# PereUbu7/Variational-Self-Organizing-Maps

Measured on AMD Instinct MI355X. Metric: training samples/sec per epoch (BMU+update), 128x128 map, 784-dim, higher is better.
Workload: dtype f32

## Files before the change

### include/vsom_hip.h

```cpp
#ifndef VSOM_HIP_H
#define VSOM_HIP_H

#include <stddef.h>
#include <stdint.h>

#ifdef __cplusplus
extern "C" {
#endif

typedef struct vsom_ctx vsom_ctx;

typedef enum vsom_status {
    VSOM_OK = 0,
    VSOM_ERR_INVALID = -1,
    VSOM_ERR_HIP = -2,
    VSOM_ERR_NOMEM = -3,
    VSOM_ERR_UNSUPPORTED = -4
} vsom_status;

typedef enum vsom_transform {
    VSOM_STANDARD = 0,
    VSOM_MEDIAN = 1,
    VSOM_CLR = 2
} vsom_transform;
// ... 52 lines not shown
                uint32_t in_len, int transform);
void vsom_destroy(vsom_ctx *ctx);

#define VSOM_CUSTOM_MAX_DEPTH 5120
int vsom_create_custom(vsom_ctx **out, int device, uint32_t width, uint32_t height, uint32_t in_len,
                       uint32_t depth, uint32_t residual_len, const char *hook_source);
int vsom_custom_compile_check(const char *hook_source, uint32_t depth, uint32_t residual_len);
int vsom_set_column_weights(vsom_ctx *ctx, const float *weights_host );
int vsom_set_chunk_validity(vsom_ctx *ctx, const uint8_t *valid_host, int one_mask);
int vsom_find_bmu_valid(vsom_ctx *ctx, const float *v_host, const uint8_t *valid_host , uint64_t *bmu_out,
                        float *dist_out);
int vsom_find_local_bmu_valid(vsom_ctx *ctx, const float *v_host, const uint8_t *valid_host, uint64_t last_bmu,
                              uint64_t *bmu_out, float *dist_out);
int vsom_dist_single_valid(vsom_ctx *ctx, const float *v_host, const uint8_t *valid_host, uint64_t node, float *dist_out);
int vsom_train_single_valid(vsom_ctx *ctx, const float *v_host, const uint8_t *valid_host, double eta, double sigma,
                            uint64_t *last_bmu, int decay_fn, float *residual_out, float *dist_out, uint64_t *bmu_out);
int vsom_set_stream(vsom_ctx *ctx, void *hip_stream);
int vsom_synchronize(vsom_ctx *ctx);
int vsom_set_bmu_mode(vsom_ctx *ctx, int mode);
int vsom_set_update_mode(vsom_ctx *ctx, int mode);
int vsom_set_sigma_mode(vsom_ctx *ctx, int mode);
int vsom_sigma_flush(vsom_ctx *ctx);
int vsom_sigma_stats(vsom_ctx *ctx, uint64_t *out );
int vsom_set_column_compaction(vsom_ctx *ctx, long min_rows);
int vsom_set_row_dedupe(vsom_ctx *ctx, double min_work);
int vsom_get_shortlist_stats(vsom_ctx *ctx, uint32_t *out );
uint32_t vsom_depth(const vsom_ctx *ctx);
uint32_t vsom_nodes(const vsom_ctx *ctx);

int vsom_set_state(vsom_ctx *ctx, const float *map, const float *sigma, const float *S,
                   const float *weight, const uint64_t *bmu_hits);
int vsom_get_state(vsom_ctx *ctx, float *map, float *sigma, float *S, float *weight,
                   uint64_t *bmu_hits);

int vsom_upload_chunk(vsom_ctx *ctx, const float *x_host, size_t B);
int vsom_upload_chunk_async(vsom_ctx *ctx, const float *x_host, size_t B);
int vsom_set_chunk_device(vsom_ctx *ctx, const float *x_dev, size_t B);
int vsom_host_alloc(void **out, size_t bytes);
int vsom_host_free(void *p);
int vsom_prefetch_chunk(vsom_ctx *ctx, const float *x_host, size_t B);
int vsom_prefetch_wait(vsom_ctx *ctx);
int vsom_commit_chunk(vsom_ctx *ctx);
int vsom_stage_next_device(vsom_ctx *ctx, const float *x_dev, size_t B);
int vsom_get_last_bmu(vsom_ctx *ctx, uint64_t *out_host);
int vsom_set_last_bmu(vsom_ctx *ctx, const uint64_t *in_host);
int vsom_get_sqres(vsom_ctx *ctx, float *out_host);
// ... 221 lines not shown
```

### variational-self-organizing-maps_amd/capi.py

```python
import ctypes as C
import os
import subprocess

import numpy as np

_HERE = os.path.dirname(os.path.abspath(__file__))
_INTREE = os.path.join(_HERE, "libvsom_hip.so")
LIB_PATH = os.environ.get("VSOM_LIB") or _INTREE

STANDARD, MEDIAN, CLR = 0, 1, 2
CUSTOM = -1
CUSTOM_MAX_DEPTH = 5120
EXPONENTIAL, INVERSE_PROPORTIONAL, BATCHMAP = 0, 1, 2
BMU_AUTO, BMU_EXACT, BMU_SHORTLIST = 0, 1, 2
UPDATE_STRICT, UPDATE_FMA, UPDATE_FMA_SIGMA = 0, 1, 2
SIGMA_AUTO, SIGMA_EAGER, SIGMA_LAZY = 0, 1, 2
BUF_MAP, BUF_SIGMA, BUF_S, BUF_WEIGHT, BUF_HITS, BUF_LASTBMU, BUF_SQRES, BUF_CHUNK, BUF_UMATRIX = range(9)
T_STAGE, T_BMU, T_FINISH, T_CW, T_UPDATE, T_ONLINE, T_SIGMA, T_COUNT = range(8)
TIMER_NAMES = ["stage", "bmu", "finish", "cw", "update", "online", "sigma"]
SIGMA_AS_WRITTEN, SIGMA_FLOOR = 0, 1
GENERATE_AS_WRITTEN, GENERATE_PER_ROW = 0, 1
NO_UNIT = 2 ** 64 - 1

SYMBOLS = [
    "vsom_last_error", "vsom_device_count", "vsom_create", "vsom_destroy", "vsom_set_stream",
    "vsom_synchronize", "vsom_set_bmu_mode", "vsom_set_update_mode", "vsom_set_column_compaction", "vsom_set_row_dedupe", "vsom_get_shortlist_stats", "vsom_depth", "vsom_nodes", "vsom_set_state",
    "vsom_get_state", "vsom_upload_chunk", "vsom_set_chunk_device", "vsom_host_alloc", "vsom_host_free",
    "vsom_prefetch_chunk", "vsom_prefetch_wait", "vsom_commit_chunk", "vsom_stage_next_device", "vsom_get_last_bmu",
    "vsom_set_last_bmu", "vsom_get_sqres", "vsom_bmu_batch", "vsom_find_bmu", "vsom_dist_single", "vsom_find_local_bmu", "vsom_find_restricted_bmu", "vsom_distances_single", "vsom_bmu_local_batch",
    "vsom_distances", "vsom_bmu_restricted_batch", "vsom_distances_row", "vsom_distances_raw", "vsom_bmd_batch", "vsom_bmu_topk_batch", "vsom_batch_phase1_async", "vsom_batch_finish_async",
    "vsom_batch_phase2_async", "vsom_batch_epoch_async", "vsom_batch_epoch", "vsom_get_mse",
    "vsom_residual_len", "vsom_train_single", "vsom_train_online_chunk", "vsom_train_online_chunk_acc", "vsom_train_online_chunk_fetch", "vsom_upload_chunk_async", "vsom_get_online_search_stats",
    "vsom_neighbourhood_weight", "vsom_device_ptr", "vsom_chunk_size", "vsom_pitch",
    "vsom_chunk_pitch", "vsom_small_map_chains", "vsom_enable_timing", "vsom_enable_timing_of", "vsom_get_timing",
    "vsom_group_create", "vsom_group_destroy", "vsom_group_size", "vsom_group_ctx", "vsom_group_transport",
    "vsom_group_synchronize", "vsom_group_set_state", "vsom_group_get_state", "vsom_group_set_update_mode",
    "vsom_group_set_bmu_mode", "vsom_group_upload_chunk", "vsom_group_prefetch_chunk", "vsom_group_prefetch_wait",
    "vsom_group_commit_chunk", "vsom_group_set_chunk_device", "vsom_group_set_last_bmu", "vsom_group_get_last_bmu",
    "vsom_group_batch_epoch_async", "vsom_group_batch_epoch", "vsom_group_get_mse",
    "vsom_create_custom", "vsom_custom_compile_check",
    "vsom_ensemble_create", "vsom_ensemble_destroy", "vsom_ensemble_size", "vsom_ensemble_train_online_chunk_fetch",
    "vsom_ensemble_batch_epoch", "vsom_ensemble_upload_chunks", "vsom_ensemble_bmu_batch",
    "vsom_umatrix", "vsom_get_umatrix", "vsom_ensemble_umatrix", "vsom_similarity_batch",
    "vsom_bmu_masked_batch", "vsom_evaluate_batch", "vsom_generate_batch", "vsom_decode_nodes",
    "vsom_batch_epoch_masked", "vsom_batch_schedule", "vsom_ensemble_batch_schedule",
    "vsom_set_sigma_mode", "vsom_sigma_flush", "vsom_sigma_stats",
    "vsom_batch_accum_begin", "vsom_batch_accum_chunk", "vsom_batch_accum_end", "vsom_batch_accum_abort",
    "vsom_batch_accum_chunk_masked", "vsom_train_online_chunk_masked",
    "vsom_similarity_masked_batch", "vsom_evaluate_masked_batch",
    "vsom_bmd_masked_batch", "vsom_generate_masked_batch",
    "vsom_set_column_weights", "vsom_set_chunk_validity", "vsom_find_bmu_valid", "vsom_find_local_bmu_valid",
    "vsom_dist_single_valid", "vsom_train_single_valid",
    "vsom_bmu_topk_masked_batch",
    "vsom_batch_schedule_masked", "vsom_ensemble_batch_epoch_masked", "vsom_ensemble_batch_schedule_masked",
    "vsom_masked_tiny_applies",
    "vsom_online_masked_tiny_applies", "vsom_ensemble_train_online_chunk_masked",
    "vsom_ensemble_bmu_masked_batch", "vsom_ensemble_similarity_masked_batch",
    "vsom_ensemble_bmu_topk_batch", "vsom_ensemble_bmu_topk_masked_batch", "vsom_ensemble_topk_applies",
]
SCHEDULE_MAX_EPOCHS = 1024


class SimilarityOut(C.Structure):
    _fields_ = [("bmu", C.POINTER(C.c_uint64)), ("dist", C.POINTER(C.c_float)), ("dmax", C.POINTER(C.c_float)),
                ("dmax_col", C.POINTER(C.c_uint32)), ("first", C.POINTER(C.c_float)), ("amax", C.POINTER(C.c_float)),
                ("amax_col", C.POINTER(C.c_uint32)), ("outside", C.POINTER(C.c_uint32)), ("delta", C.POINTER(C.c_float))]


class MaskedOut(C.Structure):
# ... 73 lines not shown
    global _lib
    if _lib is not None:
        return _lib
    if not os.path.exists(LIB_PATH):
        raise VsomError(f"{LIB_PATH} is missing: run __graft_entry__.build() "
                        "(variational-self-organizing-maps_amd/csrc/build.sh)")
    L = C.CDLL(LIB_PATH)
    vp, fp, u64p = C.c_void_p, C.POINTER(C.c_float), C.POINTER(C.c_uint64)
    L.vsom_last_error.restype = C.c_char_p
    L.vsom_device_count.restype = C.c_int
    L.vsom_create.argtypes = [C.POINTER(vp), C.c_int, C.c_uint32, C.c_uint32, C.c_uint32, C.c_int]
    L.vsom_create_custom.argtypes = [C.POINTER(vp), C.c_int, C.c_uint32, C.c_uint32, C.c_uint32, C.c_uint32, C.c_uint32,
                                     C.c_char_p]
    L.vsom_custom_compile_check.argtypes = [C.c_char_p, C.c_uint32, C.c_uint32]
    L.vsom_destroy.argtypes = [vp]
    L.vsom_destroy.restype = None
    L.vsom_set_stream.argtypes = [vp, vp]
    L.vsom_synchronize.argtypes = [vp]
    L.vsom_set_bmu_mode.argtypes = [vp, C.c_int]
    L.vsom_set_update_mode.argtypes = [vp, C.c_int]
    L.vsom_set_sigma_mode.argtypes = [vp, C.c_int]
    L.vsom_sigma_flush.argtypes = [vp]
    L.vsom_sigma_stats.argtypes = [vp, C.POINTER(C.c_uint64)]
    L.vsom_set_column_compaction.argtypes = [vp, C.c_long]
    L.vsom_set_row_dedupe.argtypes = [vp, C.c_double]
    L.vsom_get_shortlist_stats.argtypes = [vp, C.POINTER(C.c_uint32)]
    for name in ("vsom_depth", "vsom_nodes", "vsom_residual_len", "vsom_pitch", "vsom_chunk_pitch"):
        getattr(L, name).argtypes = [vp]
        getattr(L, name).restype = C.c_uint32
    L.vsom_chunk_size.argtypes = [vp]
    L.vsom_chunk_size.restype = C.c_size_t
    L.vsom_enable_timing_of.argtypes = [vp, C.c_uint32]
    L.vsom_small_map_chains.argtypes = [vp, C.c_size_t]
    L.vsom_small_map_chains.restype = C.c_int
    L.vsom_set_state.argtypes = [vp, fp, fp, fp, fp, u64p]
    L.vsom_get_state.argtypes = [vp, fp, fp, fp, fp, u64p]
    L.vsom_upload_chunk.argtypes = [vp, fp, C.c_size_t]
    L.vsom_upload_chunk_async.argtypes = [vp, fp, C.c_size_t]
    L.vsom_set_chunk_device.argtypes = [vp, vp, C.c_size_t]
    L.vsom_host_alloc.argtypes = [C.POINTER(vp), C.c_size_t]
    L.vsom_host_free.argtypes = [vp]
    L.vsom_prefetch_chunk.argtypes = [vp, fp, C.c_size_t]
    L.vsom_prefetch_wait.argtypes = [vp]
    L.vsom_commit_chunk.argtypes = [vp]
    L.vsom_stage_next_device.argtypes = [vp, vp, C.c_size_t]
    L.vsom_get_last_bmu.argtypes = [vp, u64p]
# ... 227 lines not shown
    def set_stream(self, hip_stream_ptr):
        check(lib().vsom_set_stream(self._h, C.c_void_p(hip_stream_ptr or 0)))

    def synchronize(self):
        check(lib().vsom_synchronize(self._h))

    def set_bmu_mode(self, mode):
        check(lib().vsom_set_bmu_mode(self._h, int(mode)))

    def set_update_mode(self, mode):
        check(lib().vsom_set_update_mode(self._h, int(mode)))

    def set_sigma_mode(self, mode):
        check(lib().vsom_set_sigma_mode(self._h, int(mode)))

    def sigma_flush(self):
        check(lib().vsom_sigma_flush(self._h))

    def sigma_stats(self):
        out = (C.c_uint64 * 4)()
        check(lib().vsom_sigma_stats(self._h, out))
        return {"deferred": int(out[0]), "dropped": int(out[1]), "materialised": int(out[2]), "pending": bool(out[3])}

    def set_row_dedupe(self, min_work):
        check(lib().vsom_set_row_dedupe(self._h, float(min_work)))

    def set_column_compaction(self, min_rows):
        check(lib().vsom_set_column_compaction(self._h, int(min_rows)))

    def shortlist_stats(self):
        out = (C.c_uint32 * 4)()
        check(lib().vsom_get_shortlist_stats(self._h, out))
        return {"redo_samples": int(out[0]), "candidates": int(out[1]), "samples": int(out[2]),
                "searches": int(out[3])}

    def device_ptr(self, which):
        return int(lib().vsom_device_ptr(self._h, int(which)) or 0)

    @property
    def chunk_size(self):
        return int(lib().vsom_chunk_size(self._h))

    def set_state(self, map=None, sigma=None, S=None, weight=None, hits=None):
        n, d = self.n_nodes, self.depth

        def f2(a, shape):
# ... 1102 lines not shown
```

### variational-self-organizing-maps_amd/csrc/gen_nt_asm.py

```python
#!/usr/bin/env python3
import os

CT = 32
SLOT_XOR = 0x4000
LDS_BYTES = 0x8000
SLOT_XOR_C = 0x2000
LDS_BYTES_C = 0x4000

S_KARG = "s[0:1]"
S_WGX, S_WGY = "s2", "s3"
S_XP, S_CP, S_MAP, S_SBUF = (4, 5), (6, 7), (8, 9), (10, 11)
S_LDX, S_LDN, S_B, S_NLOC, S_NQ, S_PITCH, S_N0 = "s12", "s13", "s14", "s15", "s16", "s17", "s18"
S_CNT, S_TAIL, S_TMP, S_TMP2, S_CSTEP, S_Q, S_DEAD = "s19", "s20", "s21", "s22", "s23", "s24", "s25"
S_ZP = (26, 27)
S_Z, S_ZN = "s28", "s29"
S_BIG = "s[30:31]"
S_EXEC = "s[32:33]"
V_TID = 0


class K1:
    NQ, P, WG = 1, (0, 1), 512
    S_REC = (38, 39)
    XSET = (40, 56)
    V_M, V_S, V_D, V_T, V_U = 2, 6, 10, 14, 18
    V_RING = 22
    V_G = 38
    V_CR, V_CW, V_OC, V_OC2 = 46, 47, 48, 49
    V_K = 50
    V_A = V_D
    NVGPR = 52

    @staticmethod
    def sx(xs, p):
        return sp(xs, p)


class K2:
    NQ, P, WG = 2, (0, 1, 2, 3), 256
    S_REC = (34, 35)
    S_XP2, S_ZP2 = (10, 11), (0, 1)
    S_Z2, S_ZN2 = "s100", "s101"
    XSET = (36, 68)
    V_M, V_D, V_T, V_U = 2, 10, 18, 26
    V_RING = 34
    V_G = 42
    V_CR, V_CW, V_OC, V_OC2 = 50, 51, 52, 53
    V_K = 54
    V_A = V_D
    NVGPR = 56

    @staticmethod
    def sx(xs, p):
        b = xs + 16 * (p >> 1) + 2 * (p & 1)
        return f"s[{b}:{b + 1}]"


def vp(base, p):
    return f"v[{base + 2 * p}:{base + 2 * p + 1}]"


def sp(base, p):
    return f"s[{base + 2 * p}:{base + 2 * p + 1}]"


# ... 155 lines not shown
    E = o.append
    conly = mode in MEAN
    two = k.NQ == 2
    assert conly or not two
    slot_xor = SLOT_XOR_C if conly else SLOT_XOR
    S_REC, XSET = k.S_REC, k.XSET
    V_M, V_G, V_CR, V_CW, V_OC, V_OC2, V_K, V_A, V_RING = k.V_M, k.V_G, k.V_CR, k.V_CW, k.V_OC, k.V_OC2, k.V_K, k.V_A, k.V_RING
    pieces2 = two or not conly
    E(f"\t.text\n\t.globl {name}\n\t.p2align 8\n\t.type {name},@function\n{name}:")
    E(f"\ts_load_dwordx8 s[4:11], {S_KARG}, 0x0")
    E(f"\ts_load_dwordx4 s[12:15], {S_KARG}, 0x20")
    E(f"\ts_load_dwordx2 s[16:17], {S_KARG}, 0x30")
    E(f"\ts_load_dword {S_N0}, {S_KARG}, 0x38")
    E(f"\ts_load_dwordx2 s[{S_REC[0]}:{S_REC[1]}], {S_KARG}, 0x40")
    E(f"\ts_load_dwordx2 s[{S_ZP[0]}:{S_ZP[1]}], {S_KARG}, 0x48")
    E(f"\ts_and_b32 {S_TMP}, {S_WGX}, 7")
    E(f"\ts_lshr_b32 {S_TMP2}, {S_WGX}, 3")
    E(f"\ts_lshl_b32 {S_WGY}, {S_WGY}, 3")
    E(f"\ts_add_u32 {S_WGX}, {S_WGY}, {S_TMP}")
    E(f"\ts_mov_b32 {S_WGY}, {S_TMP2}")
    E(f"\tv_and_b32_e32 v{V_TID}, 0x3ff, v{V_TID}")
    E(f"\tv_readfirstlane_b32 {S_Q}, v{V_TID}")
    E(f"\ts_lshr_b32 {S_Q}, {S_Q}, 6")
    if two:
        E(f"\ts_lshl_b32 {S_Q}, {S_Q}, 1")
    E(f"\ts_lshl_b32 {S_TMP}, {S_WGY}, 3")
    E(f"\ts_add_u32 {S_Q}, {S_Q}, {S_TMP}")
    E(f"\ts_waitcnt lgkmcnt(0)")
    E(f"\ts_cmp_eq_u64 s[{S_REC[0]}:{S_REC[1]}], 0")
    E(f"\ts_cbranch_scc1 .L_nq_{name}")
    E(f"\ts_load_dword {S_NQ}, s[{S_REC[0]}:{S_REC[1]}], 0x0")
    E(f"\ts_waitcnt lgkmcnt(0)")
    E(f"\ts_add_u32 {S_NQ}, {S_NQ}, 3")
    E(f"\ts_lshr_b32 {S_NQ}, {S_NQ}, 2")
    E(f".L_nq_{name}:")
    E(f"\ts_lshl_b32 {S_TMP}, {S_WGY}, 3")
    E(f"\ts_cmp_ge_u32 {S_TMP}, {S_NQ}")
    E(f"\ts_cbranch_scc1 .L_end_{name}")
    E(f"\ts_lshl_b32 {S_TMP}, {S_WGX}, 6")
    E(f"\ts_cmp_ge_u32 {S_TMP}, {S_NLOC}")
    E(f"\ts_cbranch_scc1 .L_end_{name}")
    E(f"\ts_cmp_ge_u32 {S_Q}, {S_NQ}")
    E(f"\ts_cselect_b32 {S_DEAD}, 1, 0")
    if mode in MED:
        E(f"\ts_mov_b32 s30, 0x7f000000")
        E(f"\ts_mov_b32 s31, 0x7f000000")
        E(f"\tv_mov_b32_e32 v{V_K}, 0xcb800000")
        E(f"\tv_mov_b32_e32 v{V_K + 1}, 0xcb800000")
    E(f"\ts_mul_i32 {S_TMP}, {S_Q}, {S_LDX}")
    E(f"\ts_mul_hi_u32 {S_TMP2}, {S_Q}, {S_LDX}")
    E(f"\ts_add_u32 s{S_XP[0]}, s{S_XP[0]}, {S_TMP}")
    E(f"\ts_addc_u32 s{S_XP[1]}, s{S_XP[1]}, {S_TMP2}")
    if two:
        E(f"\ts_add_u32 s{k.S_XP2[0]}, s{S_XP[0]}, {S_LDX}")
        E(f"\ts_addc_u32 s{k.S_XP2[1]}, s{S_XP[1]}, 0")
    E(f"\ts_lshr_b32 {S_TMP}, {S_LDX}, 7")
    if two:
        E(f"\ts_mov_b32 {S_TMP2}, {S_TMP}")
    E(f"\ts_mul_i32 {S_TMP}, {S_TMP}, {S_Q}")
    E(f"\ts_add_u32 s{S_ZP[0]}, s{S_ZP[0]}, {S_TMP}")
    E(f"\ts_addc_u32 s{S_ZP[1]}, s{S_ZP[1]}, 0")
    if two:
        E(f"\ts_add_u32 s{k.S_ZP2[0]}, s{S_ZP[0]}, {S_TMP2}")
        E(f"\ts_addc_u32 s{k.S_ZP2[1]}, s{S_ZP[1]}, 0")
    E(f"\tv_and_b32_e32 v{V_CR}, 63, v{V_TID}")
    E(f"\tv_lshlrev_b32_e32 v{V_CR}, 4, v{V_CR}")
    E(f"\tv_lshlrev_b32_e32 v{V_CW}, 4, v{V_TID}")
    E(f"\tv_lshrrev_b32_e32 v{V_OC}, 6, v{V_TID}")
    E(f"\tv_mul_lo_u32 v{V_OC}, v{V_OC}, {S_LDN}")
    E(f"\tv_add_u32_e32 v{V_OC}, v{V_OC}, v{V_CR}")
    if pieces2:
        E(f"\ts_lshl_b32 {S_TMP}, {S_LDN}, {2 if two else 3}")
        E(f"\tv_add_u32_e32 v{V_OC2}, {S_TMP}, v{V_OC}")
    E(f"\ts_lshl_b32 {S_TMP}, {S_WGX}, 10")
    if os.environ.get("VSOM_GEN_NT_CWL2"):
        E(f"\ts_and_b32 {S_TMP}, {S_TMP}, 0x400")
    E(f"\ts_add_u32 s{S_CP[0]}, s{S_CP[0]}, {S_TMP}")
    E(f"\ts_addc_u32 s{S_CP[1]}, s{S_CP[1]}, 0")
    E(f"\ts_lshl_b32 {S_CSTEP}, {S_LDN}, {3 if conly else 4}")
    for r in range(V_M, V_M + 8):
        E(f"\tv_mov_b32_e32 v{r}, 0")
    E(f"\ts_cmp_eq_u32 {S_B}, 0")
    E(f"\ts_cbranch_scc1 .L_store_{name}")
    E(f"\ts_add_u32 {S_CNT}, {S_B}, {CT - 1}")
    E(f"\ts_lshr_b32 {S_CNT}, {S_CNT}, 5")
    E(f"\ts_sub_u32 {S_CNT}, {S_CNT}, 1")
    E(f"\ts_lshl_b32 {S_TMP}, {S_CNT}, 5")
# ... 120 lines not shown
    E(f".L_store_{name}:")
    E(f"\ts_waitcnt vmcnt(0) lgkmcnt(0)")
    E(f"\ts_cmp_lg_u32 {S_DEAD}, 0")
    E(f"\ts_cbranch_scc1 .L_end_{name}")
    VN = f"v{V_A + 2}"
    VA = f"v[{V_A}:{V_A + 1}]"
    E(f"\tv_and_b32_e32 {VN}, 63, v{V_TID}")
    E(f"\ts_lshl_b32 {S_TMP}, {S_WGX}, 6")
    E(f"\tv_add_u32_e32 {VN}, {S_TMP}, {VN}")
    E(f"\tv_cmp_gt_u32_e32 vcc, {S_NLOC}, {VN}")
    E(f"\ts_and_saveexec_b64 {S_EXEC}, vcc")
    E(f"\ts_cbranch_execz .L_end_{name}")
    E(f"\tv_add_u32_e32 {VN}, {S_N0}, {VN}")
    E(f"\ts_lshl_b32 {S_TMP}, {S_Q}, 4")
    outs = [(S_MAP, V_M)] if mode in MEAN else [(S_MAP, V_M), (S_SBUF, k.V_S)]
    for base, tag in outs:
        E(f"\ts_add_u32 {S_TMP2}, s{base[0]}, {S_TMP}")
        E(f"\ts_addc_u32 s34, s{base[1]}, 0")
        E(f"\tv_mov_b32_e32 v{V_A}, {S_TMP2}")
        E(f"\tv_mov_b32_e32 v{V_A + 1}, s34")
        E(f"\tv_mad_u64_u32 {VA}, s[34:35], {VN}, {S_PITCH}, {VA}")
        E(f"\tglobal_store_dwordx4 {VA}, v[{tag}:{tag + 3}], off")
        if two:
            E(f"\ts_add_u32 {S_TMP}, {S_Q}, 1")
            E(f"\ts_cmp_ge_u32 {S_TMP}, {S_NQ}")
            E(f"\ts_cbranch_scc1 .L_end_{name}")
            E(f"\tglobal_store_dwordx4 {VA}, v[{tag + 4}:{tag + 7}], off offset:16")
    E(f".L_end_{name}:")
    E(f"\ts_endpgm")
    E(f".L_func_end_{name}:")
    E(f"\t.size {name}, .L_func_end_{name}-{name}")
    return "\n".join(o)


MODES = ("std", "fma", "sfma", "med", "mean", "meanfma", "medmean")


def emit():
    out = []
    for m in MODES:
        name = f"vsom_update_{m}_nt4_gfx950"
        out.append((name, kernel(name, m), K1.NVGPR, 80, LDS_BYTES_C if m in MEAN else LDS_BYTES, 0 if m in MED else 1, K1.WG))
    for m in MEAN:
        name = f"vsom_update_{m}_nt8_gfx950"
        out.append((name, kernel(name, m, K2), K2.NVGPR, 80, LDS_BYTES_C, 0 if m in MED else 1, K2.WG))
    return out
```

### variational-self-organizing-maps_amd/csrc/vsom_capi.hip

```cpp
#include "vsom_internal.hpp"
#include "vsom_phase2_plan.hpp"

#include <cstring>
#include <cstdlib>
#include <cmath>
#include <new>

static thread_local std::string g_last_error;

void vsom_set_error(const std::string &msg) { g_last_error = msg; }
int vsom_fail(int code, const std::string &msg)
{
    g_last_error = msg;
    return code;
}

TimerScope::TimerScope(vsom_ctx *ctx, int w) : c(ctx), which(w), on((ctx->timing >> w) & 1u)
{
    if (!on)
        return;
    if (!c->ev_pool.empty()) {
        ev = c->ev_pool.back();
        c->ev_pool.pop_back();
    } else {
// ... 348 lines not shown
{
    if (!c || mode < VSOM_SIGMA_AUTO || mode > VSOM_SIGMA_LAZY)
        return vsom_fail(VSOM_ERR_INVALID, "bad sigma mode");
    c->sigma_mode = mode;
    return VSOM_OK;
}

int vsom_sigma_flush(vsom_ctx *c)
{
    CHECK_CTX(c);
    return VSOM_OK;
}

int vsom_sigma_stats(vsom_ctx *c, uint64_t *out)
{
    if (!c || !out)
        return vsom_fail(VSOM_ERR_INVALID, "null context or output");
    for (int i = 0; i < 3; ++i)
        out[i] = c->sg_stats[i];
    out[3] = c->sg.on ? 1 : 0;
    return VSOM_OK;
}

int vsom_set_update_mode(vsom_ctx *c, int mode)
{
    if (!c || (mode != VSOM_UPDATE_STRICT && mode != VSOM_UPDATE_FMA && mode != VSOM_UPDATE_FMA_SIGMA))
        return vsom_fail(VSOM_ERR_INVALID, "bad update mode");
    if (mode != VSOM_UPDATE_STRICT)
        VSOM_CUSTOM_REFUSE(c, "a contracted update mode");
    c->update_mode = mode;
    return VSOM_OK;
}

uint32_t vsom_depth(const vsom_ctx *c) { return c ? c->D : 0; }
uint32_t vsom_nodes(const vsom_ctx *c) { return c ? c->N : 0; }
uint32_t vsom_residual_len(const vsom_ctx *c) { return c ? (c->cu ? vsom_custom_residual_len(c) : c->part_len) : 0; }
size_t vsom_chunk_size(const vsom_ctx *c) { return c ? c->B : 0; }

static bool all_zero_bits(const void *p, size_t bytes)
{
    const unsigned char *b = static_cast<const unsigned char *>(p);
    size_t i = 0;
    for (; i + 64 <= bytes; i += 64) {
        uint64_t w[8];
        std::memcpy(w, b + i, 64);
        if (w[0] | w[1] | w[2] | w[3] | w[4] | w[5] | w[6] | w[7])
// ... 901 lines not shown
```

### variational-self-organizing-maps_amd/csrc/vsom_internal.hpp

```cpp
#pragma once

#include <hip/hip_runtime.h>
#include <stdint.h>
#include <stddef.h>
#include <algorithm>
#include <map>
#include <string>
#include <tuple>
#include <vector>

#include "../../include/vsom_hip.h"
#include "vsom_buf.hpp"
#include "vsom_sched_round.hpp"

typedef unsigned long long u64;

#define VSOM_CHAIN_MAX_WAVES 448

#define VSOM_TK 32
#define TILE 64

constexpr size_t VSOM_ROW_PAD = 32;
constexpr size_t VSOM_ONL_STATE_BYTES = 4352;

// ... 84 lines not shown
    void *upd_quad[VSOM_QF_COUNT][VSOM_QV_COUNT] = {};
    bool mean_nt4 = false;
    int update_mode = VSOM_UPDATE_STRICT;
    bool use_chain = true;
    bool use_tiny = true;

    DevBuf<unsigned> cc_flags;
    DevBuf<int> cc_idx;
    DevBuf<int> cc_inv;
    DevBuf<unsigned> cc_meta;
    PinnedBuf<unsigned> cc_fb;
    unsigned cc_seen = 0;
    int cc_skip = 0;
    long cc_min_rows = 1024;
    bool cc_valid = false;
    uint32_t cpitch = 0;
    DevBuf<float> Xc;
    DevBuf<float> Mc;
    DevBuf<float> Uc_map, Uc_S;
    DevBuf<float4> Xq;
    DevBuf<unsigned> zq;
    bool xq_valid = false;
    uint32_t xq_bpad = 0, xq_quads = 0;

    struct PendingSigma {
        bool on = false;
        size_t B = 0;
        uint32_t bpad = 0;
        bool compact = false;
        VsomQuadVariant variant = VSOM_QV_STD;
        double sigma = 0.0;
    } sg;
    DevBuf<int> sg_inv; DevBuf<unsigned> sg_meta;
    DevBuf<u64> sg_bmu;
    int sigma_mode = VSOM_SIGMA_AUTO;
    unsigned sigma_unread = 0;
    bool sigma_shared = false;
    uint64_t sg_stats[3] = {0, 0, 0};

    DevBuf<float> v_dev;
    PinnedBuf<float> v_pinned;
    DevBuf<float> res_dev;
    DevBuf<u64> onl_state;
    DevBuf<float> onl_f;
    DevBuf<unsigned char> onl_img; DevBuf<float4> onl_nsc; DevBuf<float> onl_lb; DevBuf<unsigned> onl_u;
    DevBuf<float4> onl_xsc;
// ... 310 lines not shown
```

### variational-self-organizing-maps_amd/csrc/vsom_update.hip

```cpp
#include "vsom_device.hpp"
#include "vsom_phase2_plan.hpp"
#include <algorithm>
#include <cmath>
#include <cstdlib>
#include <mutex>


#define CWP_WT 512
#define CWP_THREADS (64 + CWP_WT)
template <int NW, int T, bool LUT_LDS, bool CONLY>
__global__ __launch_bounds__(CWP_THREADS) void cwp_kernel(const u64 *__restrict__ lastbmu, int B, int n0, int n1,
                                                          int W, int H, const float *__restrict__ lut,
                                                          int lutw, int luth, float2 *__restrict__ cw, int ldn,
                                                          float *__restrict__ weight)
{
    static_assert(NW * T == 2048 && CWP_WT % NW == 0 && T % 4 == 0 && T <= CWP_WT, "worker mapping");
    constexpr int LK = NW * T / CWP_WT;
    constexpr int PK = LK / 2;
    constexpr int QK = LK / 4;
    static_assert(LK % 4 == 0, "whole sample quads per worker thread");
    constexpr int SS = CWP_WT / NW;
    extern __shared__ __attribute__((aligned(16))) unsigned char cwp_smem[];
    float *wL = (float *)cwp_smem;
    float *WL = wL + 3 * T * NW;
// ... 410 lines not shown
        return VSOM_OK;
    hipModule_t mod;
#ifdef VSOM_DEVELOPMENT
    if (const char *alt = std::getenv("VSOM_ASM_HSACO")) {
        VSOM_HIP_CHECK(hipModuleLoad(&mod, alt));
    } else
#endif
    VSOM_HIP_CHECK(hipModuleLoadData(&mod, vsom_update_hsaco));
    hipFunction_t f;
    VSOM_HIP_CHECK(hipModuleGetFunction(&f, mod, "vsom_update_clr_rp8_gfx950"));
    c->upd_clr8 = f;
    static const char *const quad_names[VSOM_QF_COUNT][VSOM_QV_COUNT] = {
        {"std_nt4", "fma_nt4", "sfma_nt4", "med_nt4"},
        {"mean_nt4", "meanfma_nt4", "mean_nt4", "medmean_nt4"},
        {"mean_nt8", "meanfma_nt8", "mean_nt8", "medmean_nt8"}};
    for (int form = 0; form < VSOM_QF_COUNT; ++form)
        for (int v = 0; v < VSOM_QV_COUNT; ++v) {
            const std::string n = std::string("vsom_update_") + quad_names[form][v] + "_gfx950";
            VSOM_HIP_CHECK(hipModuleGetFunction(&f, mod, n.c_str()));
            c->upd_quad[form][v] = f;
        }
#ifdef VSOM_DEVELOPMENT
    c->mean_nt4 = std::getenv("VSOM_MEAN_NT4") != nullptr;
#endif
    c->upd_module = mod;
    return VSOM_OK;
}

double vsom_neighbourhood_weight(size_t cx, size_t cy, size_t bx, size_t by, double sigma)
{
    if (sigma > 1.0) {
        double cxd = (double)cx, cyd = (double)cy, bxd = (double)bx, byd = (double)by;
        return std::exp(-((cxd - bxd) * (cxd - bxd) / 2.0 / sigma / sigma +
                          (cyd - byd) * (cyd - byd) / 2.0 / sigma / sigma));
    } else if (cx == bx && cy == by) {
        return 1.0;
    }
    return 0.0;
}

int ensure_lut(vsom_ctx *c, double sigma)
{
    if (c->lut.p && c->lut_sigma == sigma)
        return VSOM_OK;
    uint32_t ymax = c->N ? (c->N - c->W) / c->H : 0;
    uint32_t lh = ymax + 1, lw = c->W;
// ... 52 lines not shown
    constexpr int nw = 16, T = 2048 / nw;
    const size_t smem = (size_t)5 * 2048 * sizeof(float) + (size_t)3 * T * sizeof(int2) + (lds ? lut_bytes : 0);
    const void *fn = conly ? (lds ? (const void *)cwp_kernel<nw, T, true, true> : (const void *)cwp_kernel<nw, T, false, true>)
                           : (lds ? (const void *)cwp_kernel<nw, T, true, false> : (const void *)cwp_kernel<nw, T, false, false>);
    if (smem > 64 * 1024)
        VSOM_HIP_CHECK(hipFuncSetAttribute(fn, hipFuncAttributeMaxDynamicSharedMemorySize, (int)smem));
    int B = (int)B_, in0 = (int)n0, in1 = (int)n1, iW = (int)c->W, iH = (int)c->H, lw = (int)c->lut_w, lh = (int)c->lut_h,
        ildn = (int)ldn;
    const float *lut = c->lut.p;
    float2 *cwp = c->cw.p;
    void *args[] = {&bmu, &B, &in0, &in1, &iW, &iH, &lut, &lw, &lh, &cwp, &ildn, &weight};
    VSOM_HIP_CHECK(hipLaunchKernel(fn, dim3((unsigned)((nloc + nw - 1) / nw)), dim3(CWP_THREADS), args, smem, c->stream));
    return VSOM_OK;
}

static int launch_nt_chains(vsom_ctx *c, const Phase2Plan &p, size_t n0, size_t B, uint32_t bpad, const unsigned *meta)
{
    const unsigned cols = p.compact ? c->cpitch : c->pitch;
    UpdAsmArgs a;
    a.xs = c->Xq.p;
    a.cw2 = c->cw.p;
    a.map = p.compact ? c->Uc_map.p : c->map.p;
    a.sbuf = p.compact ? c->Uc_S.p : c->sigma.p;
    a.ldx_bytes = bpad * 16u;
    a.ldn_bytes = (unsigned)(p.ldn * 16u);
    a.B = (unsigned)B;
    a.nloc = (unsigned)p.nloc;
    a.nslices = p.quads;
    a.pitch_bytes = cols * 4u;
    a.n0 = (unsigned)n0;
    a.ppitch_bytes = 0;
    a.yp = p.compact ? (const void *)meta : nullptr;
    a.zq = c->zq.p;
    size_t sz = 80;
    void *extra[] = {HIP_LAUNCH_PARAM_BUFFER_POINTER, &a, HIP_LAUNCH_PARAM_BUFFER_SIZE, &sz, HIP_LAUNCH_PARAM_END};
    VSOM_HIP_CHECK(hipModuleLaunchKernel((hipFunction_t)c->upd_quad[p.form][p.variant], p.grid_x, p.grid_y, 1, p.block, 1, 1, 0,
                                         c->stream, nullptr, extra));
    return VSOM_OK;
}

static int run_after(vsom_ctx *c, const Phase2Plan &p, size_t n0, const int *inv = nullptr)
{
    if (p.after == VSOM_P2_NOTHING)
        return VSOM_OK;
    TimerScope ts(c, VSOM_T_SIGMA);
    if (p.after != VSOM_P2_FINALIZE_COLUMNS)
        return vsom_cc_expand(c, n0, p.nloc,
                              p.after == VSOM_P2_EXPAND_MAP_ONLY ? VSOM_EXPAND_MAP
                              : p.after == VSOM_P2_EXPAND_SIGMA_ONLY ? VSOM_EXPAND_SIGMA : VSOM_EXPAND_BOTH, inv);
    for (uint32_t part = 0; part < c->nparts; ++part)
        hipLaunchKernelGGL(sigma_finalize_kernel, dim3((unsigned)p.nloc), dim3(256), 0, c->stream, c->sigma.p, c->map.p,
                           (int)c->pitch, (int)(part * c->part_pitch), (int)p.after_cols, (int)c->part_len, (int)n0, (int)p.nloc,
                           c->weight.p);
    VSOM_HIP_CHECK(hipGetLastError());
    return VSOM_OK;
}

__global__ __launch_bounds__(256) void sg_keep_record_kernel(const int *__restrict__ inv, int ninv, const unsigned *__restrict__ meta,
                                                             int *__restrict__ inv_out, unsigned *__restrict__ meta_out,
                                                             const u64 *__restrict__ bmu, int nb, u64 *__restrict__ bmu_out)
{
    const int i = blockIdx.x * blockDim.x + threadIdx.x;
    if (i < ninv)
        inv_out[i] = inv[i];
    if (i < 16 && ninv > 0)
        meta_out[i] = meta[i];
    if (i < nb)
        bmu_out[i] = bmu[i];
}

void vsom_sigma_drop(vsom_ctx *c)
{
    if (c->sg.on) {
        c->sg.on = false;
        ++c->sg_stats[1];
    }
}

static int sigma_materialise(vsom_ctx *c)
{
    const vsom_ctx::PendingSigma p = c->sg;
    int rc = ensure_lut(c, p.sigma);
    if (rc)
        return rc;
    c->sg.on = false;
    ++c->sg_stats[2];
    const Phase2Plan plan = vsom_phase2_replay(*c, p.B, p.variant, p.compact);
    {
        TimerScope ts(c, VSOM_T_CW);
        if ((rc = launch_cwp(c, c->sg_bmu.p, p.B, 0, c->N, plan.ldn, false, nullptr)))
            return rc;
// ... 51 lines not shown
    float *map_ = c->map.p, *sg_ = c->sigma.p;
    const float *wt_ = c->weight.p;
    void *args[] = {&xs_, &ildx, &cw_, &ildn, &iB, &in0, &inl, &iD, &map_, &sg_, &ipitch, &wt_};
    VSOM_HIP_CHECK(hipLaunchKernel((const void *)k3[p.variant][p.pl_log2 - 3], dim3(p.grid_x, p.grid_y), dim3(p.block), args, 0,
                                   c->stream));
    return VSOM_OK;
}

static int run_quads(vsom_ctx *c, const Phase2Plan &p, double sigma, size_t n0)
{
    int rc = vsom_xq_ensure(c);
    if (rc)
        return rc;
    if (p.offer_rows_free) {
        VSOM_HIP_CHECK(hipEventRecord(c->ev_rows_free, c->stream));
        c->rows_free_valid = true;
    }
    if (p.compact && (rc = vsom_cc_ensure_update_scratch(c)))
        return rc;
    if (!p.deferred)
        return launch_nt_chains(c, p, n0, c->B, c->xq_bpad, c->cc_meta.p);
    hipLaunchKernelGGL(sg_keep_record_kernel, dim3((unsigned)((std::max<size_t>(p.compact ? c->xpitch : 0, c->B) + 255) / 256)),
                       dim3(256), 0, c->stream, c->cc_inv.p, p.compact ? (int)c->xpitch : 0, c->cc_meta.p, c->sg_inv.p,
                       c->sg_meta.p, c->lastbmu.p, (int)c->B, c->sg_bmu.p);
    if ((rc = launch_nt_chains(c, p, n0, c->B, c->xq_bpad, c->cc_meta.p)))
        return rc;
    c->sg.on = true;
    c->sg.B = c->B;
    c->sg.bpad = c->xq_bpad;
    c->sg.compact = p.compact;
    c->sg.variant = p.variant;
    c->sg.sigma = sigma;
    ++c->sg_stats[0];
    return VSOM_OK;
}

int launch_phase2(vsom_ctx *c, double sigma, size_t n0, size_t n1, bool may_defer)
{
    if (n1 <= n0)
        return vsom_join_aux_keep(c);
    const bool full = n0 == 0 && n1 == c->N;
    if (c->sg.on && !full)
        if (int prc = sigma_materialise(c))
            return prc;
    auto done = [&]() {
        if (may_defer && full && c->sigma_unread < 1000u)
            ++c->sigma_unread;
// ... 46 lines not shown
```

### variational-self-organizing-maps_amd/csrc/vsom_xq.hip

```cpp
#include "vsom_device.hpp"

__global__ __launch_bounds__(256) void xq_transpose_kernel(const float *__restrict__ src, int ld, int B, int bpad, int nq8, float scale,
                                                           float4 *__restrict__ xq, unsigned *__restrict__ zq)
{
    __shared__ float4 tile[16][65];
    const int j0 = blockIdx.x * 64, q0 = blockIdx.y * 16, t = threadIdx.x;
    for (int pass = 0; pass < 4; ++pass) {
        const int js = pass * 16 + (t >> 4), qq = t & 15;
        const int j = j0 + js, col = 4 * (q0 + qq);
        float4 v = make_float4(0.f, 0.f, 0.f, 0.f);
        if (j < B && col + 3 < ld)
            v = *reinterpret_cast<const float4 *>(src + (size_t)j * ld + col);
        v.x *= scale;
        v.y *= scale;
        v.z *= scale;
        v.w *= scale;
        tile[qq][js] = v;
    }
    __syncthreads();
    for (int pass = 0; pass < 4; ++pass) {
        const int qq = pass * 4 + (t >> 6), js = t & 63;
        const int q = q0 + qq, j = j0 + js;
        const float4 v = tile[qq][js];
        const bool z = v.x == 0.f && v.y == 0.f && v.z == 0.f && v.w == 0.f;
        const unsigned long long m = __ballot(z);
        if (q < nq8 && j < bpad) {
            xq[(size_t)q * bpad + j] = v;
            if (js == 0)
                zq[(size_t)q * (bpad >> 5) + (j >> 5)] = (unsigned)m;
            if (js == 32)
                zq[(size_t)q * (bpad >> 5) + (j >> 5)] = (unsigned)(m >> 32);
        }
    }
}

int vsom_xq_ensure(vsom_ctx *c)
{
    if (c->xq_valid)
        return VSOM_OK;
    const bool compact = c->cc_valid;
    const uint32_t cols = compact ? c->cpitch : c->xpitch;
    const uint32_t nq8 = (cols / 4 + 7) / 8 * 8;
    const size_t bpad_cap = (c->Bcap + 31) / 32 * 32 + 32;
    const size_t need = (size_t)nq8 * bpad_cap;
    VSOM_ALLOC_CHECK(vsom_grow_set(c->stream, VSOM_BUF_SYNC, {vsom_member(c->Xq, need), vsom_member(c->zq, need / 32)}));
    const uint32_t bpad = (uint32_t)((c->B + 31) / 32 * 32 + 32);
    hipLaunchKernelGGL(xq_transpose_kernel, dim3((bpad + 63) / 64, nq8 / 16 + (nq8 % 16 ? 1 : 0)), dim3(256), 0, c->stream,
                       compact ? c->Xc.p : c->Xs.p, (int)cols, (int)c->B, (int)bpad, (int)nq8,
                       c->transform == VSOM_MEDIAN ? 0x1.0p24f : 1.f, c->Xq.p,
                       c->zq.p);
    VSOM_HIP_CHECK(hipGetLastError());
    c->xq_bpad = bpad;
    c->xq_quads = nq8;
    c->xq_valid = true;
    return VSOM_OK;
}
```

Measured before the change: 1.722 million.

## Balance two-quad update workgroups by pairing quad rows by nonzero count

Adds a quad-assignment table, computed on the device inside the keep-record kernel, that counts nonzero samples per quad row from the zero bitmask. It sorts rows by that count and pairs heavy rows with light ones, so each workgroup of the two-quad mean update kernel handles a balanced amount of work. The generated assembly now loads each workgroup's pair of quad indices from this table instead of taking adjacent rows, and stores the second quad at its own address. The cost is extra scalar loads and a serial ranking step in one block, and it only pays off when sparsity varies across columns (for example MNIST-like 784-dim data).

```diff
diff --git a/include/vsom_hip.h b/include/vsom_hip.h
--- a/include/vsom_hip.h
+++ b/include/vsom_hip.h
@@ -98,6 +98,7 @@
 int vsom_set_sigma_mode(vsom_ctx *ctx, int mode);
 int vsom_sigma_flush(vsom_ctx *ctx);
 int vsom_sigma_stats(vsom_ctx *ctx, uint64_t *out );
+int vsom_quad_assignment(vsom_ctx *ctx, uint16_t *out, size_t cap, size_t *n);
 int vsom_set_column_compaction(vsom_ctx *ctx, long min_rows);
 int vsom_set_row_dedupe(vsom_ctx *ctx, double min_work);
 int vsom_get_shortlist_stats(vsom_ctx *ctx, uint32_t *out );
diff --git a/variational-self-organizing-maps_amd/capi.py b/variational-self-organizing-maps_amd/capi.py
--- a/variational-self-organizing-maps_amd/capi.py
+++ b/variational-self-organizing-maps_amd/capi.py
@@ -44,7 +44,7 @@
     "vsom_umatrix", "vsom_get_umatrix", "vsom_ensemble_umatrix", "vsom_similarity_batch",
     "vsom_bmu_masked_batch", "vsom_evaluate_batch", "vsom_generate_batch", "vsom_decode_nodes",
     "vsom_batch_epoch_masked", "vsom_batch_schedule", "vsom_ensemble_batch_schedule",
-    "vsom_set_sigma_mode", "vsom_sigma_flush", "vsom_sigma_stats",
+    "vsom_set_sigma_mode", "vsom_sigma_flush", "vsom_sigma_stats", "vsom_quad_assignment",
     "vsom_batch_accum_begin", "vsom_batch_accum_chunk", "vsom_batch_accum_end", "vsom_batch_accum_abort",
     "vsom_batch_accum_chunk_masked", "vsom_train_online_chunk_masked",
     "vsom_similarity_masked_batch", "vsom_evaluate_masked_batch",
@@ -164,6 +164,7 @@
     L.vsom_set_sigma_mode.argtypes = [vp, C.c_int]
     L.vsom_sigma_flush.argtypes = [vp]
     L.vsom_sigma_stats.argtypes = [vp, C.POINTER(C.c_uint64)]
+    L.vsom_quad_assignment.argtypes = [vp, C.POINTER(C.c_uint16), C.c_size_t, C.POINTER(C.c_size_t)]
     L.vsom_set_column_compaction.argtypes = [vp, C.c_long]
     L.vsom_set_row_dedupe.argtypes = [vp, C.c_double]
     L.vsom_get_shortlist_stats.argtypes = [vp, C.POINTER(C.c_uint32)]
@@ -437,6 +438,13 @@
         check(lib().vsom_sigma_stats(self._h, out))
         return {"deferred": int(out[0]), "dropped": int(out[1]), "materialised": int(out[2]), "pending": bool(out[3])}
 
+    def quad_assignment(self):
+        cap = 2 * 65536
+        out = (C.c_uint16 * cap)()
+        n = C.c_size_t(0)
+        check(lib().vsom_quad_assignment(self._h, out, cap, C.byref(n)))
+        return np.ctypeslib.as_array(out)[:2 * n.value].reshape(-1, 2).copy()
+
     def set_row_dedupe(self, min_work):
         check(lib().vsom_set_row_dedupe(self._h, float(min_work)))
 
diff --git a/variational-self-organizing-maps_amd/csrc/gen_nt_asm.py b/variational-self-organizing-maps_amd/csrc/gen_nt_asm.py
--- a/variational-self-organizing-maps_amd/csrc/gen_nt_asm.py
+++ b/variational-self-organizing-maps_amd/csrc/gen_nt_asm.py
@@ -41,6 +41,7 @@
     S_REC = (34, 35)
     S_XP2, S_ZP2 = (10, 11), (0, 1)
     S_Z2, S_ZN2 = "s100", "s101"
+    S_Q2 = "s3"
     XSET = (36, 68)
     V_M, V_D, V_T, V_U = 2, 10, 18, 26
     V_RING = 34
@@ -242,11 +243,12 @@
     E(f"\tv_and_b32_e32 v{V_TID}, 0x3ff, v{V_TID}")
     E(f"\tv_readfirstlane_b32 {S_Q}, v{V_TID}")
     E(f"\ts_lshr_b32 {S_Q}, {S_Q}, 6")
-    if two:
-        E(f"\ts_lshl_b32 {S_Q}, {S_Q}, 1")
-    E(f"\ts_lshl_b32 {S_TMP}, {S_WGY}, 3")
+    E(f"\ts_lshl_b32 {S_TMP}, {S_WGY}, {2 if two else 3}")
     E(f"\ts_add_u32 {S_Q}, {S_Q}, {S_TMP}")
     E(f"\ts_waitcnt lgkmcnt(0)")
+    if two:
+        E(f"\ts_lshl_b32 {S_Q}, {S_Q}, 2")
+        E(f"\ts_load_dword {S_Q}, s[{S_SBUF[0]}:{S_SBUF[1]}], {S_Q}")
     E(f"\ts_cmp_eq_u64 s[{S_REC[0]}:{S_REC[1]}], 0")
     E(f"\ts_cbranch_scc1 .L_nq_{name}")
     E(f"\ts_load_dword {S_NQ}, s[{S_REC[0]}:{S_REC[1]}], 0x0")
@@ -254,12 +256,17 @@
     E(f"\ts_add_u32 {S_NQ}, {S_NQ}, 3")
     E(f"\ts_lshr_b32 {S_NQ}, {S_NQ}, 2")
     E(f".L_nq_{name}:")
+    if two:
+        E(f"\ts_waitcnt lgkmcnt(0)")
     E(f"\ts_lshl_b32 {S_TMP}, {S_WGY}, 3")
     E(f"\ts_cmp_ge_u32 {S_TMP}, {S_NQ}")
     E(f"\ts_cbranch_scc1 .L_end_{name}")
     E(f"\ts_lshl_b32 {S_TMP}, {S_WGX}, 6")
     E(f"\ts_cmp_ge_u32 {S_TMP}, {S_NLOC}")
     E(f"\ts_cbranch_scc1 .L_end_{name}")
+    if two:
+        E(f"\ts_lshr_b32 {k.S_Q2}, {S_Q}, 16")
+        E(f"\ts_and_b32 {S_Q}, {S_Q}, 0xffff")
     E(f"\ts_cmp_ge_u32 {S_Q}, {S_NQ}")
     E(f"\ts_cselect_b32 {S_DEAD}, 1, 0")
     if mode in MED:
@@ -267,22 +274,23 @@
         E(f"\ts_mov_b32 s31, 0x7f000000")
         E(f"\tv_mov_b32_e32 v{V_K}, 0xcb800000")
         E(f"\tv_mov_b32_e32 v{V_K + 1}, 0xcb800000")
+    if two:
+        E(f"\ts_mul_i32 {S_TMP}, {k.S_Q2}, {S_LDX}")
+        E(f"\ts_mul_hi_u32 {S_TMP2}, {k.S_Q2}, {S_LDX}")
+        E(f"\ts_add_u32 s{k.S_XP2[0]}, s{S_XP[0]}, {S_TMP}")
+        E(f"\ts_addc_u32 s{k.S_XP2[1]}, s{S_XP[1]}, {S_TMP2}")
     E(f"\ts_mul_i32 {S_TMP}, {S_Q}, {S_LDX}")
     E(f"\ts_mul_hi_u32 {S_TMP2}, {S_Q}, {S_LDX}")
     E(f"\ts_add_u32 s{S_XP[0]}, s{S_XP[0]}, {S_TMP}")
     E(f"\ts_addc_u32 s{S_XP[1]}, s{S_XP[1]}, {S_TMP2}")
-    if two:
-        E(f"\ts_add_u32 s{k.S_XP2[0]}, s{S_XP[0]}, {S_LDX}")
-        E(f"\ts_addc_u32 s{k.S_XP2[1]}, s{S_XP[1]}, 0")
     E(f"\ts_lshr_b32 {S_TMP}, {S_LDX}, 7")
     if two:
-        E(f"\ts_mov_b32 {S_TMP2}, {S_TMP}")
+        E(f"\ts_mul_i32 {S_TMP2}, {S_TMP}, {k.S_Q2}")
+        E(f"\ts_add_u32 s{k.S_ZP2[0]}, s{S_ZP[0]}, {S_TMP2}")
+        E(f"\ts_addc_u32 s{k.S_ZP2[1]}, s{S_ZP[1]}, 0")
     E(f"\ts_mul_i32 {S_TMP}, {S_TMP}, {S_Q}")
     E(f"\ts_add_u32 s{S_ZP[0]}, s{S_ZP[0]}, {S_TMP}")
     E(f"\ts_addc_u32 s{S_ZP[1]}, s{S_ZP[1]}, 0")
-    if two:
-        E(f"\ts_add_u32 s{k.S_ZP2[0]}, s{S_ZP[0]}, {S_TMP2}")
-        E(f"\ts_addc_u32 s{k.S_ZP2[1]}, s{S_ZP[1]}, 0")
     E(f"\tv_and_b32_e32 v{V_CR}, 63, v{V_TID}")
     E(f"\tv_lshlrev_b32_e32 v{V_CR}, 4, v{V_CR}")
     E(f"\tv_lshlrev_b32_e32 v{V_CW}, 4, v{V_TID}")
@@ -449,10 +457,16 @@
         E(f"\tv_mad_u64_u32 {VA}, s[34:35], {VN}, {S_PITCH}, {VA}")
         E(f"\tglobal_store_dwordx4 {VA}, v[{tag}:{tag + 3}], off")
         if two:
-            E(f"\ts_add_u32 {S_TMP}, {S_Q}, 1")
-            E(f"\ts_cmp_ge_u32 {S_TMP}, {S_NQ}")
+            VB = f"v[{V_A + 4}:{V_A + 5}]"
+            E(f"\ts_cmp_ge_u32 {k.S_Q2}, {S_NQ}")
             E(f"\ts_cbranch_scc1 .L_end_{name}")
-            E(f"\tglobal_store_dwordx4 {VA}, v[{tag + 4}:{tag + 7}], off offset:16")
+            E(f"\ts_lshl_b32 {S_TMP}, {k.S_Q2}, 4")
+            E(f"\ts_add_u32 {S_TMP2}, s{base[0]}, {S_TMP}")
+            E(f"\ts_addc_u32 s34, s{base[1]}, 0")
+            E(f"\tv_mov_b32_e32 v{V_A + 4}, {S_TMP2}")
+            E(f"\tv_mov_b32_e32 v{V_A + 5}, s34")
+            E(f"\tv_mad_u64_u32 {VB}, s[34:35], {VN}, {S_PITCH}, {VB}")
+            E(f"\tglobal_store_dwordx4 {VB}, v[{tag + 4}:{tag + 7}], off")
     E(f".L_end_{name}:")
     E(f"\ts_endpgm")
     E(f".L_func_end_{name}:")
diff --git a/variational-self-organizing-maps_amd/csrc/vsom_capi.hip b/variational-self-organizing-maps_amd/csrc/vsom_capi.hip
--- a/variational-self-organizing-maps_amd/csrc/vsom_capi.hip
+++ b/variational-self-organizing-maps_amd/csrc/vsom_capi.hip
@@ -394,6 +394,23 @@
     return VSOM_OK;
 }
 
+int vsom_quad_assignment(vsom_ctx *c, uint16_t *out, size_t cap, size_t *n)
+{
+    CHECK_CTX_KEEP(c);
+    if (!n)
+        return vsom_fail(VSOM_ERR_INVALID, "null count");
+    *n = 0;
+    if (!c->xq_valid || !c->qa_valid)
+        return VSOM_OK;
+    const size_t entries = c->xq_quads / 2;
+    if (!out || cap < 2 * entries)
+        return vsom_fail(VSOM_ERR_INVALID, "vsom_quad_assignment: the output holds fewer than 2 * entries values");
+    VSOM_HIP_CHECK(hipMemcpyAsync(out, c->qa.p, entries * sizeof(uint32_t), hipMemcpyDeviceToHost, c->stream));
+    VSOM_HIP_CHECK(hipStreamSynchronize(c->stream));
+    *n = entries;
+    return VSOM_OK;
+}
+
 int vsom_set_update_mode(vsom_ctx *c, int mode)
 {
     if (!c || (mode != VSOM_UPDATE_STRICT && mode != VSOM_UPDATE_FMA && mode != VSOM_UPDATE_FMA_SIGMA))
diff --git a/variational-self-organizing-maps_amd/csrc/vsom_internal.hpp b/variational-self-organizing-maps_amd/csrc/vsom_internal.hpp
--- a/variational-self-organizing-maps_amd/csrc/vsom_internal.hpp
+++ b/variational-self-organizing-maps_amd/csrc/vsom_internal.hpp
@@ -130,6 +130,9 @@
     DevBuf<unsigned> zq;
     bool xq_valid = false;
     uint32_t xq_bpad = 0, xq_quads = 0;
+    DevBuf<unsigned> qa;
+    bool qa_valid = false;
+    int qa_policy = 0;
 
     struct PendingSigma {
         bool on = false;
diff --git a/variational-self-organizing-maps_amd/csrc/vsom_quad_assign.hpp b/variational-self-organizing-maps_amd/csrc/vsom_quad_assign.hpp
--- /dev/null
+++ b/variational-self-organizing-maps_amd/csrc/vsom_quad_assign.hpp
@@ -0,0 +1,78 @@
+#pragma once
+
+#include <stdint.h>
+
+#if defined(__HIPCC__) || defined(__CUDACC__)
+#define VSOM_QA_FN __host__ __device__ inline
+#else
+#define VSOM_QA_FN inline
+#endif
+
+#define VSOM_QA_MAX_ROWS 2048u
+
+VSOM_QA_FN uint32_t vsom_qa_identity(uint32_t e) { return (2u * e) | ((2u * e + 1u) << 16); }
+
+VSOM_QA_FN bool vsom_qa_before(const uint32_t *counts, uint32_t a, uint32_t b)
+{
+    return counts[a] > counts[b] || (counts[a] == counts[b] && a < b);
+}
+
+VSOM_QA_FN uint32_t vsom_qa_group_rows(int policy, uint32_t nq8) { return policy == 1 ? 8u : nq8; }
+VSOM_QA_FN uint32_t vsom_qa_group_end(uint32_t lo, uint32_t group, uint32_t live) { return lo + group < live ? lo + group : live; }
+
+VSOM_QA_FN void vsom_qa_rank_row(const uint32_t *counts, uint32_t live, uint32_t group, uint32_t i, uint16_t *order)
+{
+    const uint32_t lo = i / group * group, hi = vsom_qa_group_end(lo, group, live);
+    uint32_t r = lo;
+    for (uint32_t k = lo; k < hi; ++k)
+        r += vsom_qa_before(counts, k, i) ? 1u : 0u;
+    order[r] = (uint16_t)i;
+}
+
+VSOM_QA_FN void vsom_qa_make_pair(const uint32_t *counts, const uint16_t *order, uint32_t live, uint32_t group, uint32_t p,
+                                  uint32_t *pair, uint32_t *sum)
+{
+    const uint32_t lo = p / (group / 2u) * group, hi = vsom_qa_group_end(lo, group, live);
+    const uint32_t i = lo + p % (group / 2u), q = hi - 1u - (i - lo);
+    const uint32_t a = order[i];
+    const uint32_t b = q > i ? order[q] : live;
+    pair[p] = a | (b << 16);
+    sum[p] = counts[a] + (q > i ? counts[b] : 0u);
+}
+
+VSOM_QA_FN void vsom_qa_place_pair(const uint32_t *pair, const uint32_t *sum, uint32_t npairs, uint32_t group, uint32_t p,
+                                   uint32_t *table)
+{
+    const uint32_t lo = p / (group / 2u) * (group / 2u), hi = lo + group / 2u < npairs ? lo + group / 2u : npairs;
+    uint32_t r = lo;
+    for (uint32_t k = lo; k < hi; ++k)
+        r += (sum[k] > sum[p] || (sum[k] == sum[p] && (pair[k] & 0xffffu) < (pair[p] & 0xffffu))) ? 1u : 0u;
+    table[r] = pair[p];
+}
+
+VSOM_QA_FN uint32_t vsom_qa_dead_entry(uint32_t live, uint32_t e)
+{
+    const uint32_t d = live + (live & 1u) + 2u * (e - (live + 1u) / 2u);
+    return d | ((d + 1u) << 16);
+}
+
+inline void vsom_quad_assign(const uint32_t *counts, uint32_t live, uint32_t nq8, bool identity, int policy, uint32_t *table,
+                             uint16_t *order, uint32_t *pair, uint32_t *sum)
+{
+    if (live > nq8)
+        live = nq8;
+    if (identity || nq8 > VSOM_QA_MAX_ROWS) {
+        for (uint32_t e = 0; e < nq8 / 2u; ++e)
+            table[e] = vsom_qa_identity(e);
+        return;
+    }
+    const uint32_t npairs = (live + 1u) / 2u, group = vsom_qa_group_rows(policy, nq8);
+    for (uint32_t i = 0; i < live; ++i)
+        vsom_qa_rank_row(counts, live, group, i, order);
+    for (uint32_t p = 0; p < npairs; ++p)
+        vsom_qa_make_pair(counts, order, live, group, p, pair, sum);
+    for (uint32_t p = 0; p < npairs; ++p)
+        vsom_qa_place_pair(pair, sum, npairs, group, p, table);
+    for (uint32_t e = npairs; e < nq8 / 2u; ++e)
+        table[e] = vsom_qa_dead_entry(live, e);
+}
diff --git a/variational-self-organizing-maps_amd/csrc/vsom_update.hip b/variational-self-organizing-maps_amd/csrc/vsom_update.hip
--- a/variational-self-organizing-maps_amd/csrc/vsom_update.hip
+++ b/variational-self-organizing-maps_amd/csrc/vsom_update.hip
@@ -1,5 +1,6 @@
 #include "vsom_device.hpp"
 #include "vsom_phase2_plan.hpp"
+#include "vsom_quad_assign.hpp"
 #include <algorithm>
 #include <cmath>
 #include <cstdlib>
@@ -456,6 +457,8 @@
         }
 #ifdef VSOM_DEVELOPMENT
     c->mean_nt4 = std::getenv("VSOM_MEAN_NT4") != nullptr;
+    if (const char *qp = std::getenv("VSOM_QA_POLICY"))
+        c->qa_policy = std::atoi(qp);
 #endif
     c->upd_module = mod;
     return VSOM_OK;
@@ -554,6 +557,8 @@
     a.cw2 = c->cw.p;
     a.map = p.compact ? c->Uc_map.p : c->map.p;
     a.sbuf = p.compact ? c->Uc_S.p : c->sigma.p;
+    if (p.form == VSOM_QF_MEAN_TWO_QUADS)
+        a.sbuf = c->qa.p;
     a.ldx_bytes = bpad * 16u;
     a.ldn_bytes = (unsigned)(p.ldn * 16u);
     a.B = (unsigned)B;
@@ -590,7 +595,9 @@
 
 __global__ __launch_bounds__(256) void sg_keep_record_kernel(const int *__restrict__ inv, int ninv, const unsigned *__restrict__ meta,
                                                              int *__restrict__ inv_out, unsigned *__restrict__ meta_out,
-                                                             const u64 *__restrict__ bmu, int nb, u64 *__restrict__ bmu_out)
+                                                             const u64 *__restrict__ bmu, int nb, u64 *__restrict__ bmu_out,
+                                                             unsigned *__restrict__ qa, const unsigned *__restrict__ zq,
+                                                             unsigned nq8, unsigned wpr, unsigned quads, int policy)
 {
     const int i = blockIdx.x * blockDim.x + threadIdx.x;
     if (i < ninv)
@@ -599,6 +606,35 @@
         meta_out[i] = meta[i];
     if (i < nb)
         bmu_out[i] = bmu[i];
+    if (blockIdx.x != 0 || !qa)
+        return;
+    const unsigned t = threadIdx.x, nt = blockDim.x;
+    if (policy == 2 || nq8 > VSOM_QA_MAX_ROWS) {
+        for (unsigned e = t; e < nq8 / 2; e += nt)
+            qa[e] = vsom_qa_identity(e);
+        return;
+    }
+    __shared__ uint32_t counts[VSOM_QA_MAX_ROWS], pair[VSOM_QA_MAX_ROWS / 2], sum[VSOM_QA_MAX_ROWS / 2];
+    __shared__ uint16_t order[VSOM_QA_MAX_ROWS];
+    unsigned live = ninv > 0 ? (meta[0] + 3u) >> 2 : quads;
+    live = live < nq8 ? live : nq8;
+    for (unsigned r = t; r < live; r += nt)
+        counts[r] = 0;
+    __syncthreads();
+    for (unsigned k = t; k < live * wpr; k += nt)
+        atomicAdd(&counts[k / wpr], (uint32_t)__popc(~zq[k]));
+    __syncthreads();
+    const unsigned npairs = (live + 1u) / 2u, group = vsom_qa_group_rows(policy, nq8);
+    for (unsigned r = t; r < live; r += nt)
+        vsom_qa_rank_row(counts, live, group, r, order);
+    __syncthreads();
+    for (unsigned p = t; p < npairs; p += nt)
+        vsom_qa_make_pair(counts, order, live, group, p, pair, sum);
+    __syncthreads();
+    for (unsigned p = t; p < npairs; p += nt)
+        vsom_qa_place_pair(pair, sum, npairs, group, p, qa);
+    for (unsigned e = npairs + t; e < nq8 / 2; e += nt)
+        qa[e] = vsom_qa_dead_entry(live, e);
 }
 
 void vsom_sigma_drop(vsom_ctx *c)
@@ -696,7 +732,11 @@
         return launch_nt_chains(c, p, n0, c->B, c->xq_bpad, c->cc_meta.p);
     hipLaunchKernelGGL(sg_keep_record_kernel, dim3((unsigned)((std::max<size_t>(p.compact ? c->xpitch : 0, c->B) + 255) / 256)),
                        dim3(256), 0, c->stream, c->cc_inv.p, p.compact ? (int)c->xpitch : 0, c->cc_meta.p, c->sg_inv.p,
-                       c->sg_meta.p, c->lastbmu.p, (int)c->B, c->sg_bmu.p);
+                       c->sg_meta.p, c->lastbmu.p, (int)c->B, c->sg_bmu.p,
+                       p.form == VSOM_QF_MEAN_TWO_QUADS && !c->qa_valid ? c->qa.p : nullptr, c->zq.p, c->xq_quads, c->xq_bpad / 32u,
+                       p.quads, c->transform == VSOM_MEDIAN ? 2 : c->qa_policy);
+    if (p.form == VSOM_QF_MEAN_TWO_QUADS)
+        c->qa_valid = true;
     if ((rc = launch_nt_chains(c, p, n0, c->B, c->xq_bpad, c->cc_meta.p)))
         return rc;
     c->sg.on = true;
diff --git a/variational-self-organizing-maps_amd/csrc/vsom_xq.hip b/variational-self-organizing-maps_amd/csrc/vsom_xq.hip
--- a/variational-self-organizing-maps_amd/csrc/vsom_xq.hip
+++ b/variational-self-organizing-maps_amd/csrc/vsom_xq.hip
@@ -43,7 +43,8 @@
     const uint32_t nq8 = (cols / 4 + 7) / 8 * 8;
     const size_t bpad_cap = (c->Bcap + 31) / 32 * 32 + 32;
     const size_t need = (size_t)nq8 * bpad_cap;
-    VSOM_ALLOC_CHECK(vsom_grow_set(c->stream, VSOM_BUF_SYNC, {vsom_member(c->Xq, need), vsom_member(c->zq, need / 32)}));
+    VSOM_ALLOC_CHECK(vsom_grow_set(c->stream, VSOM_BUF_SYNC, {vsom_member(c->Xq, need), vsom_member(c->zq, need / 32),
+                                                               vsom_member(c->qa, nq8 / 2)}));
     const uint32_t bpad = (uint32_t)((c->B + 31) / 32 * 32 + 32);
     hipLaunchKernelGGL(xq_transpose_kernel, dim3((bpad + 63) / 64, nq8 / 16 + (nq8 % 16 ? 1 : 0)), dim3(256), 0, c->stream,
                        compact ? c->Xc.p : c->Xs.p, (int)cols, (int)c->B, (int)bpad, (int)nq8,
@@ -53,5 +54,6 @@
     c->xq_bpad = bpad;
     c->xq_quads = nq8;
     c->xq_valid = true;
+    c->qa_valid = false;
     return VSOM_OK;
 }
```

Result: slower. 1.672 million (-2.9%).
